# revdotcom/reverb

Measured on AMD Instinct MI355X. Metric: RTFx (audio-sec/wall-sec) Reverb-ASR attention_rescoring, higher is better.
Workload: dtype bf16

## Files before the change

### reverb_amd/_lib.py

```python
from __future__ import annotations

import ctypes as C
import os

_HERE = os.path.dirname(os.path.abspath(__file__))
LIB_PATH = os.path.join(_HERE, "librvb.so")

RVB_F32, RVB_BF16, RVB_FP8 = 0, 1, 2
ACT_NONE, ACT_SILU, ACT_RELU = 0, 1, 2
NORM_LN, NORM_AFFINE = 0, 1


class RvbError(RuntimeError):
    pass


class AudioInfo(C.Structure):
    _fields_ = [("container", C.c_int32), ("sample_format", C.c_int32), ("channels", C.c_int32), ("sample_rate", C.c_int32),
                ("bits_per_sample", C.c_int32), ("md5_checked", C.c_int32), ("frames", C.c_int64), ("decode_threads", C.c_int32),
                ("reserved", C.c_int32)]


class _SizedCfg(C.Structure):

# ... 113 lines not shown
                [(n, _i32p) for n in ("q_start", "q_len", "kv_start", "kv_len", "q_pos0", "kv_index", "work")] +
                [(n, C.c_int32) for n in ("n_index", "n_work", "max_q", "q_block", "causal", "chunk", "left", "plain_order", "fold",
                                          "k_prefolded", "fold_kv_cap", "lab")] +
                [("ran", C.c_int32 * 8)])


class NormTestArgs(C.Structure):
    _fields_ = ([(n, C.c_int32) for n in ("dtype", "x_bf16", "mode", "silu", "out_f32", "out_fp8", "out2_fp8", "M", "d", "pad0")] +
                [(n, C.c_float) for n in ("eps", "eps2", "out_scale", "out2_scale")] +
                [(n, _f32p) for n in ("x", "gamma", "beta", "add", "gamma2", "beta2", "out", "out2")] +
                [("sat", C.c_uint32), ("sat2", C.c_uint32)])


_u32p = C.POINTER(C.c_uint32)

TEST_SIGNATURES = {
    "rvb_test_rownorm_ex": (C.c_int, [C.POINTER(NormTestArgs)]),
    "rvb_test_conv1_ex": (C.c_int, [C.c_int, _f32p, _f32p, _f32p, _f32p, _f32p, _f32p, C.c_int, C.c_int, C.c_int, C.c_int, C.c_float,
                                    _f32p, _u32p]),
    "rvb_test_embed": (C.c_int, [_f32p, C.c_int, _f32p, C.c_int, _i32p, _i32p, _f32p, C.c_int, C.c_int, C.c_float]),
    "rvb_test_amax_abs": (C.c_int, [C.c_int, _f32p, C.c_int64, _f32p]),
    "rvb_test_convert_f32": (C.c_int, [C.c_int, _f32p, _f32p, C.c_int64]),
    "rvb_test_gather_cache": (C.c_int, [C.c_void_p, C.c_void_p, _i32p, C.c_int, C.c_int, C.c_int, C.c_int]),
    "rvb_test_gather_pairs": (C.c_int, [_f32p, C.c_int, C.c_int64, _i32p, _i32p, C.c_int, _f32p]),
    "rvb_test_gemm": (C.c_int, [C.c_int, _f32p, _f32p, _f32p, _f32p, _f32p, C.c_int, C.c_int, C.c_int, C.c_float,
                                C.c_int, C.c_int, C.c_int, C.c_int, C.c_int, C.c_int, C.c_int]),
    "rvb_test_rownorm": (C.c_int, [C.c_int, _f32p, _f32p, _f32p, C.c_float, C.c_int, C.c_int, _f32p, _f32p, C.c_int,
                                   C.c_int, C.c_int]),
    "rvb_test_conv_block32": (C.c_int, [_f32p, _f32p, _f32p, _f32p, _f32p, _f32p, C.c_int, C.c_int, C.c_int]),
    "rvb_test_conv_s2sc": (C.c_int, [_f32p, _f32p, _f32p, _f32p, _f32p, _f32p, _f32p, C.c_int, C.c_int, C.c_int]),
    "rvb_test_conv1": (C.c_int, [C.c_int, _f32p, _f32p, _f32p, _f32p, _f32p, _f32p, C.c_int, C.c_int, C.c_int, C.c_int]),
    "rvb_test_conv_igemm_fp8": (C.c_int, [_f32p, _f32p, _f32p, _f32p, _f32p, _f32p, C.c_int, C.c_int, C.c_int, C.c_int, C.c_int, C.c_int, C.c_int,
                                           C.c_float, C.c_float, _f32p, _f32p, _f32p]),
    "rvb_test_joint_new": (C.c_void_p, [C.c_int, C.c_int, C.c_int, C.c_int, C.c_double, C.c_double, C.c_double]),
    "rvb_test_joint_free": (None, [C.c_void_p]),
    "rvb_test_joint_begin": (C.c_int, [C.c_void_p, C.c_int, _f32p, _i32p, C.c_int, C.c_float, C.c_float, _i32p, _i32p, _i32p, _i32p, _i32p,
                                       C.c_int]),
    "rvb_test_joint_finish": (C.c_int, [C.c_void_p, _f32p]),
    "rvb_test_joint_prefix": (C.c_int, [C.c_void_p, C.c_int, _i32p, _i32p]),
    "rvb_test_joint_result": (C.c_int, [C.c_void_p, _i32p, _i32p, _i32p, _f64p, _i32p, _f64p]),
    "rvb_test_glu_dwconv": (C.c_int, [C.c_int, _f32p, _f32p, _f32p, _f32p, _i32p, _f32p, C.c_int, C.c_int, C.c_int,
                                      C.c_int, C.c_int, _f32p, C.c_int]),
    "rvb_test_attention": (C.c_int, [C.c_int, _f32p, _f32p, _f32p, _f32p, _f32p, _f32p, _f32p, C.c_int, C.c_int,
                                     C.c_int, C.c_int, C.c_int, _i32p, _i32p, _i32p, _i32p, C.c_int, C.c_int]),
    "rvb_test_attention_trie": (C.c_int, [C.c_int, _f32p, _f32p, _f32p, _f32p, C.c_int, C.c_int, C.c_int, _i32p, _i32p, _i32p,
                                          _i32p, _i32p, _i32p, C.c_int, C.c_int, C.c_int]),
    "rvb_test_attention_ex": (C.c_int, [C.POINTER(AttnTestArgs)]),
    "rvb_test_attention_pos_bias": (C.c_int, [_f32p, C.c_int, C.c_int, C.c_int, C.c_int, _f32p, _f32p, C.c_int, C.c_int, C.c_float, _f32p]),
    "rvb_test_logsoftmax_topk": (C.c_int, [_f32p, C.c_int, C.c_int, C.c_int, C.c_float, C.c_int, _f32p, _i32p, _f32p]),
    "rvb_test_lse_gather": (C.c_int, [_f32p, C.c_int, C.c_int, _i32p, _f32p]),
    "rvb_test_logsoftmax_topk_ex": (C.c_int, [_f32p, C.c_int, C.c_int, C.c_int, C.c_int, C.c_float, C.c_int, _f32p, _i32p, _f32p]),
    "rvb_test_lse_gather_ex": (C.c_int, [_f32p, C.c_int, C.c_int, C.c_int, _i32p, C.c_float, C.c_int, _f32p]),
    "rvb_test_lse_gather_multi_ex": (C.c_int, [_f32p, C.c_int, C.c_int, C.c_int, _i32p, _i32p, _f32p]),
    "rvb_test_ctc_viterbi": (C.c_int, [_f32p, C.c_int, C.c_int, _i32p, C.c_int, C.c_int, C.c_int, _i32p, _f32p]),
    "rvb_test_ctc_viterbi_wild": (C.c_int, [_f32p, C.c_int, C.c_int, _f32p, C.c_float, _i32p, C.c_int, C.c_int, C.c_int, _i32p, _f32p]),
    "rvb_test_ctc_viterbi_graph": (C.c_int, [_f32p, _i32p, C.c_int, C.c_int, _f32p, C.c_float, _i32p, _i32p, _i32p, _i32p, _u8p, C.c_int,
                                             C.c_int, _i32p, _i32p, _f32p]),
    "rvb_test_ctc_score": (C.c_int, [_f32p, C.c_int, C.c_int, _i32p, C.c_int, C.c_int, C.c_int, _f64p, _f32p, _f32p, _f32p, _i32p]),
    "rvb_test_ctc_score_graph": (C.c_int, [_f32p, _i32p, C.c_int, C.c_int, _i32p, _i32p, _i32p, _i32p, _u8p, C.c_int, C.c_int, _f64p, _f32p,
                                           _f32p, _f32p, _f32p, _i32p]),
    "rvb_test_ctc_score_batch": (C.c_int, [_f32p, _i32p, C.c_int, _i32p, _i32p, C.c_int, C.c_int, C.c_int, _f64p, _f32p, _f32p, _f32p,
                                           _i32p]),
    "rvb_test_ctc_find": (C.c_int, [_f32p, _i32p, C.c_int, C.c_int, _f32p, _i32p, _i32p, C.c_int, _f32p, C.c_int, C.c_int, C.c_int, C.c_int,
                                    _i64p, _i32p, _i32p, _f32p, _i32p, _i32p, _i32p, _f32p]),
    "rvb_test_slab_windows": (C.c_int, [C.c_char_p, _i32p, _i32p, C.c_int, _i32p, C.c_int, C.c_int, _i32p, _i32p, _i32p, _i32p, _i32p]),
    "rvb_test_gemm_glu": (C.c_int, [_f32p, _f32p, _f32p, _f32p, C.c_int, C.c_int, C.c_int]),
    "rvb_test_gemm_rowadd": (C.c_int, [_f32p, _f32p, _f32p, _f32p, _f32p, C.c_int, C.c_int, C.c_int, C.c_int, C.c_int, C.c_int]),
    "rvb_test_mp3_decode": (C.c_int64, [C.c_char_p, C.c_int64, C.c_int, _f32p, C.c_int64, _i64p, _i64p, C.c_int]),
    "rvb_test_mp3_hybrid": (C.c_int, [_f32p, _f32p, C.c_int, C.c_int, _f32p]),
    "rvb_test_mp3_polyphase": (C.c_int, [_f32p, _f32p, _i32p, _f32p]),
    "rvb_test_mp3_window": (C.c_int, [_f32p]),
    "rvb_test_mp3_huffman": (C.c_int, [C.c_int, C.POINTER(C.c_uint16), C.POINTER(C.c_uint8), _i32p]),
    "rvb_test_gemm_fp8": (C.c_int, [_f32p, _f32p, _f32p, _f32p, _f32p, C.c_int, C.c_int, C.c_int, C.c_float, C.c_float, C.c_int, C.c_int,
                                    C.c_float, _f32p, _f32p]),
    "rvb_test_rownorm_fp8": (C.c_int, [_f32p, _f32p, _f32p, C.c_float, C.c_int, C.c_int, C.c_int, C.c_float, _f32p, _f32p, _f32p,
                                       C.c_float, C.c_float, _f32p, _f32p]),
    "rvb_test_lse_gather_multi": (C.c_int, [_f32p, C.c_int, C.c_int, _i32p, _i32p, C.c_int, _f32p]),
    "rvb_test_row_xent": (C.c_int, [_f32p, C.c_int, C.c_int, C.c_int, _i32p, _i32p, _f32p, _f32p, _f64p, _i32p]),
    "rvb_test_host_pool": (C.c_int, [C.c_int, C.c_int, C.c_int]),
    "rvb_test_build_trie": (C.c_int, [_i32p, _i32p, _i32p, C.c_int, C.c_int, C.c_int, C.c_int, C.c_int, _i32p, _i32p, _i32p, _i32p, _i32p, _i32p,
                                      _i32p, _i32p, _i32p, _i32p, _i32p]),
    "rvb_test_fbank": (C.c_int, [_i16p, C.c_int64, _f32p]),
    "rvb_test_fbank_ex": (C.c_int, [_i16p, _f32p, C.c_int64, _f32p]),
    "rvb_test_set_gemm_variant": (C.c_int, [C.c_int]),
    "rvb_test_set_gemm2_opts": (C.c_int, [C.c_int, C.c_int]),
    "rvb_test_gemm_timeline": (C.c_int, [C.c_int] * 6 + [C.POINTER(C.c_longlong), C.c_int, _i32p]),
    "rvb_test_gemm_bench": (C.c_int, [C.c_int, C.c_int, C.c_int, C.c_int, C.c_int, C.c_int, C.c_int, C.c_int, C.c_int,
                                      _f64p, _f64p]),
    "rvb_test_prefix_beam": (C.c_int, [_f32p, _i32p, C.c_int, C.c_int, C.c_int, _i32p, _i32p, _i32p, _i32p, _i32p,
                                       _f64p]),
    "rvb_test_prefix_beam_context": (C.c_int, [_f32p, _i32p, C.c_int, C.c_int, C.c_int, C.c_int, _i32p, _i32p, C.c_int, C.c_double,
                                               _i32p, _i32p, _i32p, _i32p, _i32p, _f64p, _f64p]),
    "rvb_test_context_walk": (C.c_int, [_i32p, _i32p, C.c_int, C.c_double, C.c_int, C.c_int, _i32p, C.c_int, _i32p, _f64p, _i32p,
                                        _f64p]),
    "rvb_test_window_stats": (C.c_int, [_f32p, C.c_int64, C.c_int64, C.c_int, C.c_int64, C.c_int, C.c_float, _f32p]),
    "rvb_test_sinc_conv": (C.c_int, [C.c_int, _f32p, C.c_int64, _f32p, C.c_int, C.c_int, C.c_int, C.c_int64, _f32p]),
    "rvb_test_pool_norm": (C.c_int, [C.c_int, C.c_int, _f32p, C.c_int, C.c_int, C.c_int, C.c_int, C.c_int, _f32p, _f32p, C.c_float,
                                     C.c_int, _f32p, C.c_int64, C.c_int64, C.c_int, _f32p, _f32p, C.c_float, C.c_float, _f32p]),
    "rvb_test_conv1d5": (C.c_int, [C.c_int, _f32p, C.c_int64, _f32p, _f32p, _f32p, C.c_int64]),
    "rvb_test_lstm_layer": (C.c_int, [C.c_int, _f32p, C.c_int, C.c_int, C.c_int, _f32p, _f32p, _f32p, _f32p, _f32p]),
    "rvb_test_classifier": (C.c_int, [C.c_int, _f32p, C.c_int, _f32p, _f32p, _f32p, C.POINTER(C.c_uint8), C.c_int64, C.c_int, C.c_int]),
    "rvb_test_tstp": (C.c_int, [C.c_int, _f32p, C.c_int, _i32p, _f32p, C.c_int, C.c_int, C.c_int, C.c_int, C.c_int, _f32p]),
    "rvb_test_conv2d": (C.c_int, [C.c_int, C.c_int, _f32p, _f32p, _f32p, _f32p, _f32p, C.c_int, C.c_int, C.c_int, C.c_int, C.c_int,
                                  C.c_int, C.c_int, C.c_int, _f32p, _f32p, C.c_int, C.c_int, C.c_int, C.c_int, _i32p]),
    "rvb_test_emb_stem": (C.c_int, [C.c_int, _f32p, C.c_int64, _i64p, C.c_int, C.c_int, C.c_int, C.c_int, C.c_int, C.c_int, _f32p, _f32p,
                                    _f32p, _f32p]),
}



class DiarCfg(_SizedCfg):
    _fields_ = [(n, C.c_int32) for n in (
        "struct_size", "dtype", "sample_rate", "window_samples", "step_samples", "sinc_filters", "sinc_channels", "lstm_hidden",
        "lstm_layers", "linear_dim", "linear_layers", "num_classes", "emb_channels", "emb_dim")]


DIAR_SIGNATURES = {
    "rvd_last_error": (C.c_char_p, []),
    "rvd_model_cfg_size": (C.c_int, []),
    "rvd_emb_windows_per_pass": (C.c_int, [_eng]),
    "rvd_create": (C.c_int, [C.POINTER(DiarCfg), C.c_int, C.POINTER(_eng)]),
    "rvd_destroy": (None, [_eng]),
    "rvd_load_tensor": (C.c_int, [_eng, C.c_char_p, _f32p, _i64p, C.c_int]),
    "rvd_finalize": (C.c_int, [_eng]),
    "rvd_num_windows": (C.c_int64, [_eng, C.c_int64]),
    "rvd_frames_per_window": (C.c_int, [_eng]),
    "rvd_upload_pcm": (C.c_int, [_eng, _i16p, C.c_int64]),
    "rvd_rerun_resident": (C.c_int, [_eng]),
    "rvd_resample_pcm": (C.c_int, [_eng, _i16p, C.c_int64, C.c_int, _i16p, _i64p]),
    "rvd_segment": (C.c_int, [_eng, C.c_int64, C.c_int, _f32p]),
    "rvd_get_classes": (C.c_int, [_eng, C.POINTER(C.c_uint8)]),
    "rvd_get_tap": (C.c_int, [_eng, C.c_char_p, _f32p]),
    "rvd_embed": (C.c_int, [_eng, _i64p, _f32p, C.c_int, _f32p]),
    "rvd_get_emb_fbank": (C.c_int, [_eng, C.c_int64, _f32p, _i32p]),
    "rvd_centroid_linkage": (C.c_int, [_eng, _f64p, C.c_int, C.c_int, _f64p]),
    "rvd_set_linkage_workgroups": (C.c_int, [_eng, C.c_int]),
    "rvd_get_emb_fp8": (C.c_int, [_eng, _i32p, _f32p, _i32p, C.POINTER(C.c_uint32)]),
    "rvd_set_emb_fp8_scales": (C.c_int, [_eng, _f32p, C.c_int32]),
    "rvd_set_profiling": (C.c_int, [_eng, C.c_int]),
    "rvd_reset_timings": (C.c_int, [_eng]),
    "rvd_get_timing": (C.c_int, [_eng, C.c_char_p, _f64p, _f64p, _i64p]),
}

_lib = None
_test_lib = None
TEST_LIB_PATH = os.path.join(_HERE, "librvb_test.so")


def load_test():
    global _test_lib
    if _test_lib is not None:
        return _test_lib
    if not os.path.exists(TEST_LIB_PATH):
        raise RvbError(f"{TEST_LIB_PATH} not found: run `python -m reverb_amd.build` (hipcc, gfx950)")
    lib = C.CDLL(TEST_LIB_PATH)
    for name, (res, args) in list(SIGNATURES.items()) + list(DIAR_SIGNATURES.items()) + list(TEST_SIGNATURES.items()):
        fn = getattr(lib, name)
        fn.restype = res
        fn.argtypes = args
    _test_lib = lib
    return lib


def load():
    global _lib
    if os.environ.get("RVB_LAB") == "1":
# ... 49 lines not shown
```

### reverb_amd/csrc/engine.hip

```cpp
#include "engine.h"

#include <algorithm>
#include <atomic>
#include <condition_variable>
#include <functional>
#include <mutex>
#include <chrono>
#include <cmath>
#include <cstdlib>
#include <cstring>
#include <thread>

namespace rvb {

static thread_local std::string g_err;
void set_error(const std::string& msg) { g_err = msg; }
const char* last_error() { return g_err.c_str(); }

int DevBuf::ensure(size_t n) {
  if (n <= bytes && p) return OK;
  if (p) { (void)hipFree(p); p = nullptr; bytes = 0; }
  if (n == 0) n = 16;
  hipError_t err = hipMalloc(&p, n);
  if (err != hipSuccess) {
// ... 2690 lines not shown
  RVB_HIP_CHECK(hipMemcpyAsync(raw.data(), e->d_f8sat.p, raw.size() * 4, hipMemcpyDeviceToHost, e->stream));
  if (reset) RVB_HIP_CHECK(hipMemsetAsync(e->d_f8sat.p, 0, (e->enc.size() + 1) * 8 * 4, e->stream));
  RVB_HIP_CHECK(hipStreamSynchronize(e->stream));
  if (counts)
    for (size_t l = 0; l < e->enc.size(); ++l)
      for (int k = 0; k < 7; ++k) counts[l * 7 + k] = raw[l * 8 + k];
  return OK;
}
int rvb_get_fp8_subsample(rvb_engine* e, float* scale, uint32_t* clipped, int reset) {
  if (!e) { set_error("rvb_get_fp8_subsample: null engine"); return E_ARG; }
  if (!e->fp8) { set_error("rvb_get_fp8_subsample: not an RVB_FP8 engine"); return E_STATE; }
  if (scale) *scale = e->f8_state == 2 ? e->f8_x1 : 0.f;
  if (clipped) *clipped = 0;
  if (e->d_f8sat.p && (clipped || reset)) {
    unsigned* slot = e->d_f8sat.as<unsigned>() + e->enc.size() * 8 + 1;
    uint32_t v = 0;
    RVB_HIP_CHECK(hipMemcpyAsync(&v, slot, 4, hipMemcpyDeviceToHost, e->stream));
    if (reset) RVB_HIP_CHECK(hipMemsetAsync(slot, 0, 4, e->stream));
    RVB_HIP_CHECK(hipStreamSynchronize(e->stream));
    if (clipped) *clipped = v;
  }
  return OK;
}
int rvb_set_fp8_scales(rvb_engine* e, const float* scales, int32_t n) {
  if (!e || !scales) { set_error("rvb_set_fp8_scales: null argument"); return E_ARG; }
  if (!e->fp8) { set_error("rvb_set_fp8_scales: not an RVB_FP8 engine"); return E_STATE; }
  const int32_t nb7 = (int32_t)(e->enc.size() * 7);
  if (!e->finalized || (n != nb7 && n != nb7 + 1)) {
    set_error("rvb_set_fp8_scales: need 7 scales per conformer block of a finalized engine (+ optionally the subsampling scale, as rvb_get_fp8_scales returns them)");
    return E_ARG;
  }
  for (int i = 0; i < nb7; ++i) if (!(scales[i] > 0.f) || !std::isfinite(scales[i])) { set_error("rvb_set_fp8_scales: scales must be positive and finite"); return E_ARG; }
  if (n == nb7 + 1) {
    if (!(scales[nb7] >= 0.f) || !std::isfinite(scales[nb7])) { set_error("rvb_set_fp8_scales: the subsampling scale must be >= 0 and finite"); return E_ARG; }
    e->f8_x1 = scales[nb7];
  }
  e->f8.resize(e->enc.size());
  for (size_t l = 0; l < e->enc.size(); ++l) {
    const float* v = scales + l * 7;
    e->f8[l] = {v[0], v[1], v[2], v[3], v[4], v[5], v[6]};
  }
  if (e->f8_groups.size() != e->enc.size()) RVB_TRY(set_fp8_policy_impl(e, -1, 0, -1));
  e->f8_state = 2;
  RVB_HIP_CHECK(hipSetDevice(e->device));
  RVB_TRY(reset_f8sat(e));
  return OK;
}
int rvb_get_rescore_stats(rvb_engine* e, int64_t* decoder_rows, int64_t* pairs) {
  if (!e) { set_error("rvb_get_rescore_stats: null engine"); return E_ARG; }
  if (decoder_rows) *decoder_rows = e->rescore_rows;
  if (pairs) *pairs = e->rescore_pairs;
  return OK;
}
int rvb_get_rescore_logp(rvb_engine* e, int chunk, int hyp, int right, float* out) {
  if (!e || !out || chunk < 0 || chunk >= (int)e->rescored.size()) { set_error("rvb_get_rescore_logp: bad chunk"); return E_STATE; }
  const RescoreResult& r = e->rescored[chunk];
  const auto& v = right ? r.rlogp : r.logp;
  if (hyp < 0 || hyp >= (int)v.size()) { set_error("rvb_get_rescore_logp: bad hyp"); return E_ARG; }
  for (size_t i = 0; i < v[hyp].size(); ++i) out[i] = v[hyp][i];
  return OK;
}

int rvb_set_profiling(rvb_engine* e, int level) { if (!e) return E_ARG; drain_prof(e); e->profiling = (level == 1 || level == 2) ? level : 0; return OK; }
int rvb_reset_timings(rvb_engine* e) { if (!e) return E_ARG; drain_prof(e); e->prof.clear(); return OK; }
int rvb_get_timing(rvb_engine* e, const char* name, double* ms, double* flops, int64_t* launches) {
  if (!e || !name) return E_ARG;
  drain_prof(e);
  auto it = e->prof.find(name);
  ProfEntry pe; if (it != e->prof.end()) pe = it->second;
  if (ms) *ms = pe.ms; if (flops) *flops = pe.flops; if (launches) *launches = pe.launches;
  return OK;
}
int rvb_get_timing_bytes(rvb_engine* e, const char* name, double* bytes) {
  if (!e || !name || !bytes) return E_ARG;
  auto it = e->prof.find(name);
  *bytes = it != e->prof.end() ? it->second.bytes : 0.0;
  return OK;
}

}

#ifdef RVB_TEST_API
#include "test_api.h"
extern "C" int rvb_test_build_trie(const int32_t* tokens, const int32_t* lens, const int32_t* chunk_of, int n_hyps, int n_chunks, int sos,
                                   int eos, int reversed, int32_t* n_rows, int32_t* tok, int32_t* pos, int32_t* path, int32_t* hq_start,
                                   int32_t* hq_len, int32_t* hq_pos0, int32_t* tgt_ptr, int32_t* tgt, int32_t* pair_slot, int32_t* n_work) {
  if (!tokens || !lens || !chunk_of || !n_rows || n_hyps < 0) { set_error("rvb_test_build_trie: bad argument"); return E_ARG; }
  std::vector<HypRef> hyps;
  std::vector<int> first(n_hyps);
  int P = 0, off = 0;
  for (int i = 0; i < n_hyps; ++i) { hyps.push_back({chunk_of[i], i, lens[i], P}); first[i] = off; P += lens[i] + 1; off += lens[i]; }
  TrieBatch t;
  auto seq = [&](const HypRef& h, int j) { return tokens[first[h.idx] + (reversed ? h.len - 1 - j : j)]; };
  build_trie_range(hyps.data(), hyps.data() + hyps.size(), 0, n_chunks, sos, eos, seq, &t);
  {
    std::vector<TrieBatch> part(std::max(n_chunks, 0));
    size_t a = 0;
    for (int b = 0; b < n_chunks; ++b) {
      size_t z = a;
      while (z < hyps.size() && hyps[z].chunk == b) ++z;
      build_trie_range(hyps.data() + a, hyps.data() + z, b, 1, sos, eos, seq, &part[b]);
      a = z;
    }
    TrieBatch m;
    merge_tries(part, &m);
    const bool same = m.R == t.R && m.P == t.P && m.max_chunk_rows == t.max_chunk_rows && m.tok == t.tok && m.pos == t.pos &&
                      m.path == t.path && m.hq_start == t.hq_start && m.hq_len == t.hq_len && m.hq_pos0 == t.hq_pos0 &&
                      m.hkv_start == t.hkv_start && m.hkv_len == t.hkv_len && m.crow_start == t.crow_start &&
                      m.crow_len == t.crow_len && m.tgt_ptr == t.tgt_ptr && m.tgt == t.tgt && m.pair_slot == t.pair_slot &&
                      m.work == t.work;
    if (a != hyps.size() || !same) {
      std::string which;
#define RVB_DIFF(f) if (!(m.f == t.f)) which += std::string(" ") + #f;
      RVB_DIFF(R) RVB_DIFF(P) RVB_DIFF(max_chunk_rows) RVB_DIFF(tok) RVB_DIFF(pos) RVB_DIFF(path) RVB_DIFF(hq_start) RVB_DIFF(hq_len)
      RVB_DIFF(hq_pos0) RVB_DIFF(hkv_start) RVB_DIFF(hkv_len) RVB_DIFF(crow_start) RVB_DIFF(crow_len) RVB_DIFF(tgt_ptr) RVB_DIFF(tgt)
      RVB_DIFF(pair_slot) RVB_DIFF(work)
#undef RVB_DIFF
      set_error("rvb_test_build_trie: the stitched per-chunk tries differ from the batch trie in:" + which);
      return E_STATE;
    }
  }
  *n_rows = t.R;
  if (n_work) *n_work = (int32_t)t.work.size() / 2;
  auto cp = [](int32_t* dst, const std::vector<int32_t>& v) { if (dst) memcpy(dst, v.data(), v.size() * 4); };
  cp(tok, t.tok); cp(pos, t.pos); cp(path, t.path); cp(hq_start, t.hq_start); cp(hq_len, t.hq_len); cp(hq_pos0, t.hq_pos0);
  cp(tgt_ptr, t.tgt_ptr); cp(tgt, t.tgt); cp(pair_slot, t.pair_slot);
  return OK;
}

extern "C" int rvb_test_host_pool(int n_threads, int items, int rounds) {
  if (n_threads < 1 || items < 0 || rounds < 1) { set_error("rvb_test_host_pool: bad argument"); return E_ARG; }
  HostPool pool;
  std::vector<std::atomic<int>> hits(items);
  for (int r = 0; r < rounds; ++r) {
    for (auto& h : hits) h.store(0);
    std::atomic<int> next(0), entered(0);
    const unsigned n = (unsigned)std::max(1, n_threads - (r % 3));
    pool.run(n, [&] {
      entered.fetch_add(1);
      for (int i = next.fetch_add(1); i < items; i = next.fetch_add(1)) hits[i].fetch_add(1);
    });
    if (entered.load() != (int)n) { set_error("rvb_test_host_pool: a job was not run by the requested number of threads"); return E_STATE; }
    for (int i = 0; i < items; ++i)
      if (hits[i].load() != 1) { set_error("rvb_test_host_pool: work item executed " + std::to_string(hits[i].load()) + " times"); return E_STATE; }
  }
  return OK;
}

extern "C" int rvb_test_fbank_ex(const int16_t* pcm, const float* wave, int64_t n_samples, float* feats) {
  if ((pcm == nullptr) == (wave == nullptr) || !feats || n_samples < 0) { set_error("rvb_test_fbank_ex: one of pcm / wave, feats and n_samples >= 0 are needed"); return E_ARG; }
  int ndev = 0;
  if (hipGetDeviceCount(&ndev) != hipSuccess || ndev <= 0) { set_error("no HIP device available: librvb has no CPU fallback"); return E_HIP; }
  rvb_engine e;
  RVB_TRY(make_fbank_tables(&e));
  const int64_t nf = rvb_num_frames(n_samples);
  const size_t in_bytes = (size_t)n_samples * (pcm ? 2 : 4), out_bytes = (size_t)(nf + 4) * 80 * 4;
  void* din = nullptr;
  DevBuf df;
  int r = df.ensure(out_bytes);
  if (r == OK && in_bytes && hipMalloc(&din, in_bytes) != hipSuccess) { set_error("rvb_test_fbank_ex: hipMalloc failed"); r = E_NOMEM; }
  if (r == OK && in_bytes && hipMemcpy(din, pcm ? (const void*)pcm : (const void*)wave, in_bytes, hipMemcpyHostToDevice) != hipSuccess) { set_error("rvb_test_fbank_ex: upload failed"); r = E_HIP; }
  if (r == OK && hipMemset(df.p, 0xff, out_bytes) != hipSuccess) { set_error("rvb_test_fbank_ex: memset failed"); r = E_HIP; }
  FbankTables t{e.fb_window.as<float>(), e.fb_twiddle.as<float>(), e.fb_melw.as<float>(), e.fb_lo.as<int>(), e.fb_hi.as<int>()};
  if (r == OK) r = pcm ? fbank(nullptr, (const int16_t*)din, nf, df.as<float>(), t) : fbank_f32(nullptr, (const float*)din, nf, df.as<float>(), t);
  if (r == OK && hipDeviceSynchronize() != hipSuccess) { set_error("fbank kernel failed"); r = E_HIP; }
  if (r == OK && hipMemcpy(feats, df.p, out_bytes, hipMemcpyDeviceToHost) != hipSuccess) { set_error("rvb_test_fbank_ex: download failed"); r = E_HIP; }
  if (din) (void)hipFree(din);
  df.release();
  for (DevBuf* b : {&e.fb_window, &e.fb_twiddle, &e.fb_melw, &e.fb_lo, &e.fb_hi}) b->release();
  return r;
}

extern "C" int rvb_test_fbank(const int16_t* pcm, int64_t n_samples, float* feats) {
  if (!pcm || !feats || n_samples < 0) { set_error("rvb_test_fbank: null argument"); return E_ARG; }
  const int64_t nf = rvb_num_frames(n_samples);
  std::vector<float> all((size_t)(nf + 4) * 80);
  RVB_TRY(rvb_test_fbank_ex(pcm, nullptr, n_samples, all.data()));
  memcpy(feats, all.data(), (size_t)nf * 80 * 4);
  return OK;
}
#endif
```

### reverb_amd/csrc/fbank.hip

```cpp
#include <algorithm>
#include <cmath>
#include <vector>

#include "../../include/rvb.h"
#include "common.h"
#include "kernels.h"

namespace rvb {

static constexpr int WIN = 400, SHIFT = 160, NFFT = 512, NBIN = 257, NMEL = 80;

template <typename In>
__global__ __launch_bounds__(256) void fbank_kernel(const In* __restrict__ pcm, int64_t n_frames,
                                                    float* __restrict__ feats, FbankTables t) {
  __shared__ float s_re[4][NFFT];
  __shared__ float s_im[4][NFFT];
  const int lane = threadIdx.x & 63;
  const int w = threadIdx.x >> 6;
  const int64_t frame = (int64_t)blockIdx.x * 4 + w;
  const bool live = frame < n_frames;
  float* re = s_re[w];
  float* im = s_im[w];

  float x[7];
  float sum = 0.f;
  const In* src = pcm + frame * SHIFT;
#pragma unroll
  for (int i = 0; i < 7; ++i) {
    const int j = lane + 64 * i;
    x[i] = (live && j < WIN) ? (float)src[j] : 0.f;
    sum += x[i];
  }
  const float mean = wave_sum(sum) / (float)WIN;
#pragma unroll
  for (int i = 0; i < 7; ++i) {
    const int j = lane + 64 * i;
    if (j < WIN) im[j] = x[i] - mean;
  }
  __syncthreads();
  float y[8];
#pragma unroll
  for (int i = 0; i < 8; ++i) {
    const int j = lane + 64 * i;
    float v = 0.f;
    if (j < WIN) {
      const float cur = im[j];
      const float prev = im[j > 0 ? j - 1 : 0];
      v = (cur - 0.97f * prev) * t.window[j];
    }
    y[i] = v;
  }
  __syncthreads();
#pragma unroll
  for (int i = 0; i < 8; ++i) {
    const int j = lane + 64 * i;
    re[__brev((unsigned)j) >> 23] = y[i];
    im[j] = 0.f;
  }
  __syncthreads();
#pragma unroll 1
  for (int s = 0; s < 9; ++s) {
    const int half = 1 << s;
#pragma unroll
    for (int q = 0; q < 4; ++q) {
      const int b = lane + 64 * q;
      const int j = b & (half - 1);
      const int i0 = ((b >> s) << (s + 1)) + j;
      const int i1 = i0 + half;
      const int tw = j << (8 - s);
      const float wr = t.twiddle[2 * tw], wi = t.twiddle[2 * tw + 1];
      const float ar = re[i0], ai = im[i0], br = re[i1], bi = im[i1];
      const float tr = wr * br - wi * bi;
      const float ti = wr * bi + wi * br;
      re[i0] = ar + tr; im[i0] = ai + ti;
      re[i1] = ar - tr; im[i1] = ai - ti;
    }
    __syncthreads();
  }
  float pw[5];
#pragma unroll
  for (int i = 0; i < 5; ++i) {
    const int j = lane + 64 * i;
    pw[i] = (j < NBIN) ? re[j] * re[j] + im[j] * im[j] : 0.f;
  }
  __syncthreads();
#pragma unroll
  for (int i = 0; i < 5; ++i) {
    const int j = lane + 64 * i;
    if (j < NBIN) re[j] = pw[i];
  }
  __syncthreads();
  if (live) {
#pragma unroll
    for (int i = 0; i < 2; ++i) {
      const int m = lane + 64 * i;
      if (m < NMEL) {
        const int lo = t.mel_lo[m], hi = t.mel_hi[m];
        const float* wrow = t.mel_w + (size_t)m * NBIN;
        float acc = 0.f;
        for (int b = lo; b < hi; ++b) acc += re[b] * wrow[b];
        feats[frame * NMEL + m] = logf(fmaxf(acc, 1.1920928955078125e-07f));
      }
    }
  }
}

int fbank(hipStream_t s, const int16_t* pcm, int64_t n_frames, float* feats, const FbankTables& t) {
  if (n_frames <= 0) return OK;
  hipLaunchKernelGGL(fbank_kernel<int16_t>, dim3(cdiv(n_frames, 4)), dim3(256), 0, s, pcm, n_frames, feats, t);
  RVB_HIP_CHECK(hipGetLastError());
  return OK;
}

int fbank_f32(hipStream_t s, const float* wave, int64_t n_frames, float* feats, const FbankTables& t) {
  if (n_frames <= 0) return OK;
  hipLaunchKernelGGL(fbank_kernel<float>, dim3(cdiv(n_frames, 4)), dim3(256), 0, s, wave, n_frames, feats, t);
  RVB_HIP_CHECK(hipGetLastError());
  return OK;
}

template <typename In>
__global__ __launch_bounds__(256) void resample_kernel(const In* __restrict__ pcm, int64_t n_in, const float* __restrict__ ker,
                                                       int orig, int new_, int width, int K, float* __restrict__ out,
                                                       int64_t n_out) {
  const int64_t n = (int64_t)blockIdx.x * 256 + threadIdx.x;
  if (n >= n_out) return;
  const int64_t j = n / new_;
  const int p = (int)(n - j * new_);
  const int64_t base = j * orig - width;
  const float* kr = ker + (size_t)p * K;
  float acc = 0.f;
  for (int k = 0; k < K; ++k) {
    const int64_t i = base + k;
    if (i >= 0 && i < n_in) acc = fmaf(kr[k], (float)pcm[i], acc);
  }
  out[n] = acc;
}
int resample(hipStream_t s, const int16_t* pcm, int64_t n_in, const float* ker, int orig, int new_, int width, int K, float* out,
             int64_t n_out) {
  if (n_out <= 0) return OK;
  hipLaunchKernelGGL(resample_kernel<int16_t>, dim3(cdiv(n_out, 256)), dim3(256), 0, s, pcm, n_in, ker, orig, new_, width, K, out, n_out);
  RVB_HIP_CHECK(hipGetLastError());
  return OK;
}

int resample_f32(hipStream_t s, const float* pcm, int64_t n_in, const float* ker, int orig, int new_, int width, int K, float* out,
             int64_t n_out) {
  if (n_out <= 0) return OK;
  hipLaunchKernelGGL(resample_kernel<float>, dim3(cdiv(n_out, 256)), dim3(256), 0, s, pcm, n_in, ker, orig, new_, width, K, out, n_out);
  RVB_HIP_CHECK(hipGetLastError());
  return OK;
}

void resample_taps(int sample_rate, int target, std::vector<float>* ker, int* orig_out, int* new_out, int* width_out, int* K_out) {
  int a = sample_rate, b = target;
  while (b) { const int t = a % b; a = b; b = t; }
  const int orig = sample_rate / a, nw = target / a;
  const double lpw = 6.0, rolloff = 0.99;
  const double base_freq = std::min(orig, nw) * rolloff;
  const int width = (int)std::ceil(lpw * orig / base_freq);
  const int K = 2 * width + orig;
  ker->assign((size_t)nw * K, 0.f);
  const double PI = 3.14159265358979323846;
  for (int p = 0; p < nw; ++p)
    for (int k = 0; k < K; ++k) {
      double t = (-(double)p / nw + (double)(k - width) / orig) * base_freq;
      t = std::max(-lpw, std::min(lpw, t));
      const double c = std::cos(t * PI / lpw / 2.0);
      const double window = c * c;
      t *= PI;
      const double sinc = t == 0.0 ? 1.0 : std::sin(t) / t;
      (*ker)[(size_t)p * K + k] = (float)(sinc * window * (base_freq / orig));
    }
  *orig_out = orig; *new_out = nw; *width_out = width; *K_out = K;
}

struct FbankAny { int win, shift, nmel; };
__global__ __launch_bounds__(256) void fbank_any_kernel(const float* __restrict__ wave, int64_t n_frames, float* __restrict__ feats,
                                                        FbankTables t, FbankAny g) {
  __shared__ float s_re[4][NFFT];
  __shared__ float s_im[4][NFFT];
  const int lane = threadIdx.x & 63;
  const int w = threadIdx.x >> 6;
  const int64_t frame = (int64_t)blockIdx.x * 4 + w;
  const bool live = frame < n_frames;
  float* re = s_re[w];
  float* im = s_im[w];
  float x[8];
  float sum = 0.f;
  const float* src = wave + frame * g.shift;
#pragma unroll
  for (int i = 0; i < 8; ++i) {
    const int j = lane + 64 * i;
    x[i] = (live && j < g.win) ? src[j] : 0.f;
    sum += x[i];
  }
  const float mean = wave_sum(sum) / (float)g.win;
#pragma unroll
  for (int i = 0; i < 8; ++i) {
// ... 148 lines not shown
```

Baseline: 27600.

## Rewrite fbank kernel as register radix-8 FFT with persistent frame loop

Rebuilds the fbank kernel so that each wavefront runs the 512-point FFT as three radix-8 passes held in registers. Data moves between passes through padded LDS rows guarded by wavefront-level fences, replacing nine block-wide __syncthreads stages. Pre-emphasis now uses lane shuffles, and window, twiddle and mel weights are held in registers or LDS. The grid is capped and each block loops over frames, prefetching the next frame's samples. The old kernel is kept in a lab header for test comparison, and the disabled fp contraction is there to keep numerics close to the original.

```diff
diff --git a/reverb_amd/_lib.py b/reverb_amd/_lib.py
--- a/reverb_amd/_lib.py
+++ b/reverb_amd/_lib.py
@@ -219,6 +219,7 @@
                                       _i32p, _i32p, _i32p, _i32p, _i32p]),
     "rvb_test_fbank": (C.c_int, [_i16p, C.c_int64, _f32p]),
     "rvb_test_fbank_ex": (C.c_int, [_i16p, _f32p, C.c_int64, _f32p]),
+    "rvb_test_fbank_v1_ex": (C.c_int, [_i16p, _f32p, C.c_int64, _f32p]),
     "rvb_test_set_gemm_variant": (C.c_int, [C.c_int]),
     "rvb_test_set_gemm2_opts": (C.c_int, [C.c_int, C.c_int]),
     "rvb_test_gemm_timeline": (C.c_int, [C.c_int] * 6 + [C.POINTER(C.c_longlong), C.c_int, _i32p]),
diff --git a/reverb_amd/csrc/engine.hip b/reverb_amd/csrc/engine.hip
--- a/reverb_amd/csrc/engine.hip
+++ b/reverb_amd/csrc/engine.hip
@@ -2796,6 +2796,7 @@
 
 #ifdef RVB_TEST_API
 #include "test_api.h"
+#include "lab_v1.h"
 extern "C" int rvb_test_build_trie(const int32_t* tokens, const int32_t* lens, const int32_t* chunk_of, int n_hyps, int n_chunks, int sos,
                                    int eos, int reversed, int32_t* n_rows, int32_t* tok, int32_t* pos, int32_t* path, int32_t* hq_start,
                                    int32_t* hq_len, int32_t* hq_pos0, int32_t* tgt_ptr, int32_t* tgt, int32_t* pair_slot, int32_t* n_work) {
@@ -2861,8 +2862,8 @@
   return OK;
 }
 
-extern "C" int rvb_test_fbank_ex(const int16_t* pcm, const float* wave, int64_t n_samples, float* feats) {
-  if ((pcm == nullptr) == (wave == nullptr) || !feats || n_samples < 0) { set_error("rvb_test_fbank_ex: one of pcm / wave, feats and n_samples >= 0 are needed"); return E_ARG; }
+static int fbank_lab(const char* who, bool first_form, const int16_t* pcm, const float* wave, int64_t n_samples, float* feats) {
+  if ((pcm == nullptr) == (wave == nullptr) || !feats || n_samples < 0) { set_error(std::string(who) + ": one of pcm / wave, feats and n_samples >= 0 are needed"); return E_ARG; }
   int ndev = 0;
   if (hipGetDeviceCount(&ndev) != hipSuccess || ndev <= 0) { set_error("no HIP device available: librvb has no CPU fallback"); return E_HIP; }
   rvb_engine e;
@@ -2872,17 +2873,25 @@
   void* din = nullptr;
   DevBuf df;
   int r = df.ensure(out_bytes);
-  if (r == OK && in_bytes && hipMalloc(&din, in_bytes) != hipSuccess) { set_error("rvb_test_fbank_ex: hipMalloc failed"); r = E_NOMEM; }
-  if (r == OK && in_bytes && hipMemcpy(din, pcm ? (const void*)pcm : (const void*)wave, in_bytes, hipMemcpyHostToDevice) != hipSuccess) { set_error("rvb_test_fbank_ex: upload failed"); r = E_HIP; }
-  if (r == OK && hipMemset(df.p, 0xff, out_bytes) != hipSuccess) { set_error("rvb_test_fbank_ex: memset failed"); r = E_HIP; }
+  if (r == OK && in_bytes && hipMalloc(&din, in_bytes) != hipSuccess) { set_error(std::string(who) + ": hipMalloc failed"); r = E_NOMEM; }
+  if (r == OK && in_bytes && hipMemcpy(din, pcm ? (const void*)pcm : (const void*)wave, in_bytes, hipMemcpyHostToDevice) != hipSuccess) { set_error(std::string(who) + ": upload failed"); r = E_HIP; }
+  if (r == OK && hipMemset(df.p, 0xff, out_bytes) != hipSuccess) { set_error(std::string(who) + ": memset failed"); r = E_HIP; }
   FbankTables t{e.fb_window.as<float>(), e.fb_twiddle.as<float>(), e.fb_melw.as<float>(), e.fb_lo.as<int>(), e.fb_hi.as<int>()};
-  if (r == OK) r = pcm ? fbank(nullptr, (const int16_t*)din, nf, df.as<float>(), t) : fbank_f32(nullptr, (const float*)din, nf, df.as<float>(), t);
+  if (r == OK && first_form) r = pcm ? v1::fbank(nullptr, (const int16_t*)din, nf, df.as<float>(), t) : v1::fbank_f32(nullptr, (const float*)din, nf, df.as<float>(), t);
+  else if (r == OK) r = pcm ? fbank(nullptr, (const int16_t*)din, nf, df.as<float>(), t) : fbank_f32(nullptr, (const float*)din, nf, df.as<float>(), t);
   if (r == OK && hipDeviceSynchronize() != hipSuccess) { set_error("fbank kernel failed"); r = E_HIP; }
-  if (r == OK && hipMemcpy(feats, df.p, out_bytes, hipMemcpyDeviceToHost) != hipSuccess) { set_error("rvb_test_fbank_ex: download failed"); r = E_HIP; }
+  if (r == OK && hipMemcpy(feats, df.p, out_bytes, hipMemcpyDeviceToHost) != hipSuccess) { set_error(std::string(who) + ": download failed"); r = E_HIP; }
   if (din) (void)hipFree(din);
   df.release();
   for (DevBuf* b : {&e.fb_window, &e.fb_twiddle, &e.fb_melw, &e.fb_lo, &e.fb_hi}) b->release();
   return r;
+}
+
+extern "C" int rvb_test_fbank_ex(const int16_t* pcm, const float* wave, int64_t n_samples, float* feats) {
+  return fbank_lab("rvb_test_fbank_ex", false, pcm, wave, n_samples, feats);
+}
+extern "C" int rvb_test_fbank_v1_ex(const int16_t* pcm, const float* wave, int64_t n_samples, float* feats) {
+  return fbank_lab("rvb_test_fbank_v1_ex", true, pcm, wave, n_samples, feats);
 }
 
 extern "C" int rvb_test_fbank(const int16_t* pcm, int64_t n_samples, float* feats) {
diff --git a/reverb_amd/csrc/fbank.hip b/reverb_amd/csrc/fbank.hip
--- a/reverb_amd/csrc/fbank.hip
+++ b/reverb_amd/csrc/fbank.hip
@@ -10,111 +10,182 @@
 
 static constexpr int WIN = 400, SHIFT = 160, NFFT = 512, NBIN = 257, NMEL = 80;
 
+static constexpr int FB_ROW = 72, FB_LDS = 8 * FB_ROW;
+static constexpr int FB_W0 = 10, FB_W1 = 16;
+static constexpr int FB_MAX_GRID = 2048;
+
+__device__ inline void fb_lds_fence() {
+  __builtin_amdgcn_fence(__ATOMIC_ACQ_REL, "wavefront");
+  __builtin_amdgcn_wave_barrier();
+}
+
+__device__ inline void fb_stages(float (&re)[8], float (&im)[8], const float (&wr)[7], const float (&wi)[7]) {
+#pragma clang fp contract(off)
+#pragma unroll
+  for (int u = 0; u < 3; ++u) {
+#pragma unroll
+    for (int r = 0; r < 8; ++r) {
+      if ((r >> u) & 1) continue;
+      const int k = (1 << u) - 1 + (r & ((1 << u) - 1)), r1 = r | (1 << u);
+      const float ar = re[r], ai = im[r], br = re[r1], bi = im[r1];
+      const float tr = __builtin_fmaf(wr[k], br, -(wi[k] * bi));
+      const float ti = __builtin_fmaf(wi[k], br, wr[k] * bi);
+      re[r] = ar + tr; im[r] = ai + ti;
+      re[r1] = ar - tr; im[r1] = ai - ti;
+    }
+  }
+}
+
+__device__ inline void fb_twiddles(const float* __restrict__ tw, int s0, int jlow, int width, float (&wr)[7], float (&wi)[7]) {
+#pragma unroll
+  for (int u = 0; u < 3; ++u) {
+#pragma unroll
+    for (int sel = 0; sel < (1 << u); ++sel) {
+      const int k = (1 << u) - 1 + sel;
+      const int idx = (jlow + width * sel) << (8 - (s0 + u));
+      wr[k] = tw[2 * idx]; wi[k] = tw[2 * idx + 1];
+    }
+  }
+}
+
+template <typename In> struct FbRaw { typedef In type; };
+template <> struct FbRaw<int16_t> { typedef unsigned type; };
+__device__ inline float fb_raw(float v) { return v; }
+__device__ inline unsigned fb_raw(int16_t v) { return (unsigned short)v; }
+__device__ inline float fb_sample(float r) { return r; }
+__device__ inline float fb_sample(unsigned r) { return (float)(int16_t)(unsigned short)r; }
+
 template <typename In>
 __global__ __launch_bounds__(256) void fbank_kernel(const In* __restrict__ pcm, int64_t n_frames,
                                                     float* __restrict__ feats, FbankTables t) {
-  __shared__ float s_re[4][NFFT];
-  __shared__ float s_im[4][NFFT];
+#pragma clang fp contract(off)
+  __shared__ __align__(16) float s_re[4][FB_LDS];
+  __shared__ __align__(16) float s_im[4][FB_LDS];
   const int lane = threadIdx.x & 63;
   const int w = threadIdx.x >> 6;
-  const int64_t frame = (int64_t)blockIdx.x * 4 + w;
-  const bool live = frame < n_frames;
-  float* re = s_re[w];
-  float* im = s_im[w];
-
-  float x[7];
-  float sum = 0.f;
-  const In* src = pcm + frame * SHIFT;
-#pragma unroll
-  for (int i = 0; i < 7; ++i) {
-    const int j = lane + 64 * i;
-    x[i] = (live && j < WIN) ? (float)src[j] : 0.f;
-    sum += x[i];
-  }
-  const float mean = wave_sum(sum) / (float)WIN;
-#pragma unroll
-  for (int i = 0; i < 7; ++i) {
-    const int j = lane + 64 * i;
-    if (j < WIN) im[j] = x[i] - mean;
-  }
-  __syncthreads();
-  float y[8];
-#pragma unroll
-  for (int i = 0; i < 8; ++i) {
-    const int j = lane + 64 * i;
-    float v = 0.f;
-    if (j < WIN) {
-      const float cur = im[j];
-      const float prev = im[j > 0 ? j - 1 : 0];
-      v = (cur - 0.97f * prev) * t.window[j];
-    }
-    y[i] = v;
-  }
-  __syncthreads();
-#pragma unroll
-  for (int i = 0; i < 8; ++i) {
-    const int j = lane + 64 * i;
-    re[__brev((unsigned)j) >> 23] = y[i];
-    im[j] = 0.f;
-  }
-  __syncthreads();
-#pragma unroll 1
-  for (int s = 0; s < 9; ++s) {
-    const int half = 1 << s;
-#pragma unroll
-    for (int q = 0; q < 4; ++q) {
-      const int b = lane + 64 * q;
-      const int j = b & (half - 1);
-      const int i0 = ((b >> s) << (s + 1)) + j;
-      const int i1 = i0 + half;
-      const int tw = j << (8 - s);
-      const float wr = t.twiddle[2 * tw], wi = t.twiddle[2 * tw + 1];
-      const float ar = re[i0], ai = im[i0], br = re[i1], bi = im[i1];
-      const float tr = wr * br - wi * bi;
-      const float ti = wr * bi + wi * br;
-      re[i0] = ar + tr; im[i0] = ai + ti;
-      re[i1] = ar - tr; im[i1] = ai - ti;
-    }
-    __syncthreads();
-  }
-  float pw[5];
-#pragma unroll
-  for (int i = 0; i < 5; ++i) {
-    const int j = lane + 64 * i;
-    pw[i] = (j < NBIN) ? re[j] * re[j] + im[j] * im[j] : 0.f;
-  }
-  __syncthreads();
-#pragma unroll
-  for (int i = 0; i < 5; ++i) {
-    const int j = lane + 64 * i;
-    if (j < NBIN) re[j] = pw[i];
-  }
-  __syncthreads();
-  if (live) {
-#pragma unroll
-    for (int i = 0; i < 2; ++i) {
-      const int m = lane + 64 * i;
-      if (m < NMEL) {
-        const int lo = t.mel_lo[m], hi = t.mel_hi[m];
-        const float* wrow = t.mel_w + (size_t)m * NBIN;
-        float acc = 0.f;
-        for (int b = lo; b < hi; ++b) acc += re[b] * wrow[b];
-        feats[frame * NMEL + m] = logf(fmaxf(acc, 1.1920928955078125e-07f));
-      }
-    }
-  }
-}
+  float* re_s = s_re[w];
+  float* im_s = s_im[w];
+  __shared__ float s_tw[512];
+  __shared__ float s_mw1[(NMEL - 64) * (FB_W1 + 1)];
+  for (int i = threadIdx.x; i < 512; i += 256) s_tw[i] = t.twiddle[i];
+  if (threadIdx.x < (NMEL - 64) * FB_W1) {
+    const int m = threadIdx.x / FB_W1, b = threadIdx.x % FB_W1, lo = t.mel_lo[64 + m];
+    s_mw1[m * (FB_W1 + 1) + b] = lo + b < t.mel_hi[64 + m] ? t.mel_w[(size_t)(64 + m) * NBIN + lo + b] : 0.f;
+  }
+  __syncthreads();
+  const int64_t stride = (int64_t)gridDim.x * 4;
+  int64_t frame = (int64_t)blockIdx.x * 4 + w;
+  if (frame >= n_frames) return;
+
+  float win[7];
+#pragma unroll
+  for (int i = 0; i < 7; ++i) { const int j = lane + 64 * i; win[i] = j < WIN ? t.window[j] : 0.f; }
+  float wrA[7], wiA[7], wrB[7], wiB[7];
+  fb_twiddles(t.twiddle, 0, 0, 1, wrA, wiA);
+  fb_twiddles(t.twiddle, 3, lane & 7, 8, wrB, wiB);
+  const bool two = lane < NMEL - 64;
+  const int lo0 = t.mel_lo[lane], n0 = t.mel_hi[lane] - lo0;
+  const int lo1 = two ? t.mel_lo[64 + lane] : 0, n1 = two ? t.mel_hi[64 + lane] - lo1 : 0;
+  const float* wrow0 = t.mel_w + (size_t)lane * NBIN + lo0;
+  const float* wrow1 = t.mel_w + (size_t)(two ? 64 + lane : 0) * NBIN + lo1;
+  float mw0[FB_W0];
+#pragma unroll
+  for (int b = 0; b < FB_W0; ++b) mw0[b] = b < n0 ? wrow0[b] : 0.f;
+  const float* mw1 = s_mw1 + (two ? lane : 0) * (FB_W1 + 1);
+  const int prev_lane = (lane + 63) & 63;
+  const int src_lane = (int)(__brev((unsigned)lane) >> 26);
+  const int offA = lane * 8 + (lane >> 3) * 8;
+  const int offB = (lane >> 3) * FB_ROW + (lane & 7);
+  const int offC = lane;
+
+  typedef typename FbRaw<In>::type Raw;
+  Raw x[7];
+  auto load = [&](int64_t f, Raw (&v)[7]) {
+    const In* src = pcm + f * SHIFT;
+#pragma unroll
+    for (int i = 0; i < 7; ++i) { const int j = lane + 64 * i; v[i] = j < WIN ? fb_raw(src[j]) : (Raw)0; }
+  };
+  load(frame, x);
+  for (; frame < n_frames; frame += stride) {
+    float d[7];
+    float sum = 0.f;
+#pragma unroll
+    for (int i = 0; i < 7; ++i) { d[i] = fb_sample(x[i]); sum += d[i]; }
+    load(frame + stride < n_frames ? frame + stride : frame, x);
+    const float mean = wave_sum(sum) / (float)WIN;
+#pragma unroll
+    for (int i = 0; i < 7; ++i) d[i] -= mean;
+    float y[7];
+    float below = d[0];
+#pragma unroll
+    for (int i = 0; i < 7; ++i) {
+      const float left = __shfl(d[i], prev_lane, 64);
+      const float prev = lane > 0 ? left : below;
+      below = left;
+      y[i] = lane + 64 * i < WIN ? win[i] * __builtin_fmaf(-0.97f, prev, d[i]) : 0.f;
+    }
+    float re[8], im[8];
+#pragma unroll
+    for (int r = 0; r < 8; ++r) {
+      const int i = ((r & 1) << 2) | (r & 2) | (r >> 2);
+      re[r] = i < 7 ? __shfl(y[i < 7 ? i : 0], src_lane, 64) : 0.f;
+      im[r] = 0.f;
+    }
+    fb_stages(re, im, wrA, wiA);
+    fb_lds_fence();
+    *(float4*)(re_s + offA) = make_float4(re[0], re[1], re[2], re[3]);
+    *(float4*)(re_s + offA + 4) = make_float4(re[4], re[5], re[6], re[7]);
+    *(float4*)(im_s + offA) = make_float4(im[0], im[1], im[2], im[3]);
+    *(float4*)(im_s + offA + 4) = make_float4(im[4], im[5], im[6], im[7]);
+    fb_lds_fence();
+#pragma unroll
+    for (int r = 0; r < 8; ++r) { re[r] = re_s[offB + 8 * r]; im[r] = im_s[offB + 8 * r]; }
+    fb_stages(re, im, wrB, wiB);
+    fb_lds_fence();
+#pragma unroll
+    for (int r = 0; r < 8; ++r) { re_s[offB + 8 * r] = re[r]; im_s[offB + 8 * r] = im[r]; }
+    fb_lds_fence();
+#pragma unroll
+    for (int r = 0; r < 8; ++r) { re[r] = re_s[offC + FB_ROW * r]; im[r] = im_s[offC + FB_ROW * r]; }
+    {
+      float wrC[7], wiC[7];
+      fb_twiddles(s_tw, 6, lane, 64, wrC, wiC);
+      fb_stages(re, im, wrC, wiC);
+    }
+    fb_lds_fence();
+#pragma unroll
+    for (int r = 0; r < 4; ++r) re_s[64 * r + lane] = __builtin_fmaf(re[r], re[r], im[r] * im[r]);
+    if (lane == 0) re_s[256] = re[4] * re[4] + im[4] * im[4];
+    fb_lds_fence();
+    {
+      float acc = 0.f;
+#pragma unroll
+      for (int b = 0; b < FB_W0; ++b) { const float p = re_s[lo0 + b]; acc = __builtin_fmaf(b < n0 ? p : 0.f, mw0[b], acc); }
+      for (int b = FB_W0; b < n0; ++b) acc = __builtin_fmaf(re_s[lo0 + b], wrow0[b], acc);
+      feats[frame * NMEL + lane] = logf(fmaxf(acc, 1.1920928955078125e-07f));
+    }
+    if (two) {
+      float acc = 0.f;
+#pragma unroll
+      for (int b = 0; b < FB_W1; ++b) { const float p = re_s[lo1 + b]; acc = __builtin_fmaf(b < n1 ? p : 0.f, mw1[b], acc); }
+      for (int b = FB_W1; b < n1; ++b) acc = __builtin_fmaf(re_s[lo1 + b], wrow1[b], acc);
+      feats[frame * NMEL + 64 + lane] = logf(fmaxf(acc, 1.1920928955078125e-07f));
+    }
+  }
+}
+
+static int fbank_grid(int64_t n_frames) { return (int)std::min<int64_t>(cdiv(n_frames, 4), FB_MAX_GRID); }
 
 int fbank(hipStream_t s, const int16_t* pcm, int64_t n_frames, float* feats, const FbankTables& t) {
   if (n_frames <= 0) return OK;
-  hipLaunchKernelGGL(fbank_kernel<int16_t>, dim3(cdiv(n_frames, 4)), dim3(256), 0, s, pcm, n_frames, feats, t);
+  hipLaunchKernelGGL(fbank_kernel<int16_t>, dim3(fbank_grid(n_frames)), dim3(256), 0, s, pcm, n_frames, feats, t);
   RVB_HIP_CHECK(hipGetLastError());
   return OK;
 }
 
 int fbank_f32(hipStream_t s, const float* wave, int64_t n_frames, float* feats, const FbankTables& t) {
   if (n_frames <= 0) return OK;
-  hipLaunchKernelGGL(fbank_kernel<float>, dim3(cdiv(n_frames, 4)), dim3(256), 0, s, wave, n_frames, feats, t);
+  hipLaunchKernelGGL(fbank_kernel<float>, dim3(fbank_grid(n_frames)), dim3(256), 0, s, wave, n_frames, feats, t);
   RVB_HIP_CHECK(hipGetLastError());
   return OK;
 }
diff --git a/reverb_amd/csrc/lab_v1.h b/reverb_amd/csrc/lab_v1.h
--- /dev/null
+++ b/reverb_amd/csrc/lab_v1.h
@@ -0,0 +1,121 @@
+#ifndef RVB_LAB_V1_H_
+#define RVB_LAB_V1_H_
+#include "common.h"
+#include "kernels.h"
+
+namespace rvb {
+namespace v1 {
+
+static constexpr int WIN = 400, SHIFT = 160, NFFT = 512, NBIN = 257, NMEL = 80;
+
+template <typename In>
+__global__ __launch_bounds__(256) void fbank_kernel_v1(const In* __restrict__ pcm, int64_t n_frames,
+                                                    float* __restrict__ feats, FbankTables t) {
+  __shared__ float s_re[4][NFFT];
+  __shared__ float s_im[4][NFFT];
+  const int lane = threadIdx.x & 63;
+  const int w = threadIdx.x >> 6;
+  const int64_t frame = (int64_t)blockIdx.x * 4 + w;
+  const bool live = frame < n_frames;
+  float* re = s_re[w];
+  float* im = s_im[w];
+
+  float x[7];
+  float sum = 0.f;
+  const In* src = pcm + frame * SHIFT;
+#pragma unroll
+  for (int i = 0; i < 7; ++i) {
+    const int j = lane + 64 * i;
+    x[i] = (live && j < WIN) ? (float)src[j] : 0.f;
+    sum += x[i];
+  }
+  const float mean = wave_sum(sum) / (float)WIN;
+#pragma unroll
+  for (int i = 0; i < 7; ++i) {
+    const int j = lane + 64 * i;
+    if (j < WIN) im[j] = x[i] - mean;
+  }
+  __syncthreads();
+  float y[8];
+#pragma unroll
+  for (int i = 0; i < 8; ++i) {
+    const int j = lane + 64 * i;
+    float v = 0.f;
+    if (j < WIN) {
+      const float cur = im[j];
+      const float prev = im[j > 0 ? j - 1 : 0];
+      v = (cur - 0.97f * prev) * t.window[j];
+    }
+    y[i] = v;
+  }
+  __syncthreads();
+#pragma unroll
+  for (int i = 0; i < 8; ++i) {
+    const int j = lane + 64 * i;
+    re[__brev((unsigned)j) >> 23] = y[i];
+    im[j] = 0.f;
+  }
+  __syncthreads();
+#pragma unroll 1
+  for (int s = 0; s < 9; ++s) {
+    const int half = 1 << s;
+#pragma unroll
+    for (int q = 0; q < 4; ++q) {
+      const int b = lane + 64 * q;
+      const int j = b & (half - 1);
+      const int i0 = ((b >> s) << (s + 1)) + j;
+      const int i1 = i0 + half;
+      const int tw = j << (8 - s);
+      const float wr = t.twiddle[2 * tw], wi = t.twiddle[2 * tw + 1];
+      const float ar = re[i0], ai = im[i0], br = re[i1], bi = im[i1];
+      const float tr = wr * br - wi * bi;
+      const float ti = wr * bi + wi * br;
+      re[i0] = ar + tr; im[i0] = ai + ti;
+      re[i1] = ar - tr; im[i1] = ai - ti;
+    }
+    __syncthreads();
+  }
+  float pw[5];
+#pragma unroll
+  for (int i = 0; i < 5; ++i) {
+    const int j = lane + 64 * i;
+    pw[i] = (j < NBIN) ? re[j] * re[j] + im[j] * im[j] : 0.f;
+  }
+  __syncthreads();
+#pragma unroll
+  for (int i = 0; i < 5; ++i) {
+    const int j = lane + 64 * i;
+    if (j < NBIN) re[j] = pw[i];
+  }
+  __syncthreads();
+  if (live) {
+#pragma unroll
+    for (int i = 0; i < 2; ++i) {
+      const int m = lane + 64 * i;
+      if (m < NMEL) {
+        const int lo = t.mel_lo[m], hi = t.mel_hi[m];
+        const float* wrow = t.mel_w + (size_t)m * NBIN;
+        float acc = 0.f;
+        for (int b = lo; b < hi; ++b) acc += re[b] * wrow[b];
+        feats[frame * NMEL + m] = logf(fmaxf(acc, 1.1920928955078125e-07f));
+      }
+    }
+  }
+}
+
+inline int fbank(hipStream_t s, const int16_t* pcm, int64_t n_frames, float* feats, const FbankTables& t) {
+  if (n_frames <= 0) return OK;
+  hipLaunchKernelGGL(fbank_kernel_v1<int16_t>, dim3(cdiv(n_frames, 4)), dim3(256), 0, s, pcm, n_frames, feats, t);
+  RVB_HIP_CHECK(hipGetLastError());
+  return OK;
+}
+inline int fbank_f32(hipStream_t s, const float* wave, int64_t n_frames, float* feats, const FbankTables& t) {
+  if (n_frames <= 0) return OK;
+  hipLaunchKernelGGL(fbank_kernel_v1<float>, dim3(cdiv(n_frames, 4)), dim3(256), 0, s, wave, n_frames, feats, t);
+  RVB_HIP_CHECK(hipGetLastError());
+  return OK;
+}
+
+}
+}
+#endif
```

Result: no change. 27670 (median of 2 runs) (+0.3%).
